# nkb-tech/nkb-classification

Hardware: AMD Instinct MI355X
Metric: images/sec train step (3x224x224) (higher is better)
Workload: dtype bf16; 1 GPU; resnet50 single-task train step, 1000 classes, bs=256/GPU, bf16 compute + fp32 master weights, NAdam, 3x224x224; global_batch=256, parallelism=dp1

## Files before the change

nkb-classification_amd/csrc/elementwise.hip:

```cpp
#include "common.h"
#include <stdlib.h>
#include <atomic>

static inline unsigned grid_for(size_t work_items, int block = 256, unsigned cap = 256 * 16) {
    size_t g = (work_items + block - 1) / block;
    if (g > cap) g = cap;
    if (g < 1) g = 1;
    return (unsigned)g;
}

template <typename T> struct Chunk;
template <> struct Chunk<bf16_t> {
    static constexpr int N = 8;
    __device__ static __forceinline__ void load(const bf16_t* p, float* f) { unpack8(*(const u32x4*)p, f); }
    __device__ static __forceinline__ void store(bf16_t* p, const float* f) { *(u32x4*)p = pack8(f); }
};
template <> struct Chunk<float> {
    static constexpr int N = 4;
    __device__ static __forceinline__ void load(const float* p, float* f) {
        const f32x4 v = *(const f32x4*)p;
        f[0] = v[0]; f[1] = v[1]; f[2] = v[2]; f[3] = v[3];
    }
    __device__ static __forceinline__ void store(float* p, const float* f) { *(f32x4*)p = (f32x4){f[0], f[1], f[2], f[3]}; }
};

static inline int env_int(const char* name, int dflt) {
    const char* v = getenv(name);
    return v && *v ? atoi(v) : dflt;
}
#ifndef NKB_BN_FUSED
#define NKB_BN_FUSED 1
#endif
static constexpr int g_bn_fused = NKB_BN_FUSED;

template <int NC>
__device__ __forceinline__ void ldvec(const float* __restrict__ p, float* o) {
#pragma unroll
    for (int i = 0; i < NC / 4; ++i) {
        const f32x4 v = *(const f32x4*)(p + 4 * i);
        o[4 * i] = v[0]; o[4 * i + 1] = v[1]; o[4 * i + 2] = v[2]; o[4 * i + 3] = v[3];
    }
}

static inline int bn_partitions(int C) { return C <= 128 ? 64 : (C <= 256 ? 32 : 16); }
template <bool WT>
__device__ __forceinline__ void bn_partial_reduce_body(const float* __restrict__ partials, int tiles, int C, double* __restrict__ dpart,
                                                       double (&red)[2][16][64]) {
    const int cx = threadIdx.x & 63, py = threadIdx.x >> 6;
    const int c = blockIdx.x * 64 + cx;
    double s = 0.0, ss = 0.0;
    if (c < C) {
        for (int t = blockIdx.y * 16 + py; t < tiles; t += 16 * (int)gridDim.y) {
            s += (double)partials[((size_t)t * 2) * C + c];
            ss += (double)partials[((size_t)t * 2 + 1) * C + c];
        }
    }
    red[0][py][cx] = s;
    red[1][py][cx] = ss;
    __syncthreads();
    if (py != 0 || c >= C) return;
    s = 0.0; ss = 0.0;
    for (int k = 0; k < 16; ++k) { s += red[0][k][cx]; ss += red[1][k][cx]; }
    double* d0 = dpart + ((size_t)blockIdx.y * 2) * C + c;
    double* d1 = dpart + ((size_t)blockIdx.y * 2 + 1) * C + c;
    if constexpr (WT) {
        __hip_atomic_store(d0, s, __ATOMIC_RELAXED, __HIP_MEMORY_SCOPE_AGENT);
        __hip_atomic_store(d1, ss, __ATOMIC_RELAXED, __HIP_MEMORY_SCOPE_AGENT);
    } else {
        *d0 = s; *d1 = ss;
    }
}
__global__ void bn_partial_reduce_kernel(const float* __restrict__ partials, int tiles, int C, double* __restrict__ dpart) {
    __shared__ double red[2][16][64];
    bn_partial_reduce_body<false>(partials, tiles, C, dpart, red);
}

__device__ unsigned g_bn_tickets[128 * 32];
__device__ __forceinline__ bool bn_arrive_last(unsigned* ticket, unsigned parts) {
    __shared__ unsigned last_flag;
    asm volatile("s_waitcnt vmcnt(0)" ::: "memory");
    __syncthreads();
    if (threadIdx.x == 0) {
        const unsigned t = __hip_atomic_fetch_add(ticket, 1u, __ATOMIC_RELAXED, __HIP_MEMORY_SCOPE_AGENT);
        const bool last = t == parts - 1;
        if (last) {
            __hip_atomic_store(ticket, 0u, __ATOMIC_RELAXED, __HIP_MEMORY_SCOPE_AGENT);
            __builtin_amdgcn_fence(__ATOMIC_ACQUIRE, "agent");
            asm volatile("s_waitcnt vmcnt(0)" ::: "memory");
        }
        last_flag = last ? 1u : 0u;
    }
    __syncthreads();
    return last_flag != 0u;
}
static unsigned* bn_ticket_slot(int cols) {
    static std::atomic<unsigned> next{0};
    if (cols > 32) return nullptr;
    unsigned* base = nullptr;
    if (hipGetSymbolAddress((void**)&base, HIP_SYMBOL(g_bn_tickets)) != hipSuccess || !base) return nullptr;
    return base + (next.fetch_add(1u) % 128u) * 32u;
}

template <typename PT>
__device__ __forceinline__ void bn_finalize_body(const PT* __restrict__ partials, int tiles, int C, float count,
                                                 const float* __restrict__ gamma, const float* __restrict__ beta,
                                                 float* __restrict__ running_mean, float* __restrict__ running_var,
                                                 float momentum, float eps, int training, float* __restrict__ scale,
                                                 float* __restrict__ shift, float* __restrict__ save_mean,
                                                 float* __restrict__ save_invstd, double (&red)[2][16][64]) {
    const int cx = threadIdx.x & 63, py = threadIdx.x >> 6;
    const int c = blockIdx.x * 64 + cx;
    double s = 0.0, ss = 0.0;
    if (training && c < C) {
        for (int t = py; t < tiles; t += 16) {
            s += (double)partials[((size_t)t * 2) * C + c];
            ss += (double)partials[((size_t)t * 2 + 1) * C + c];
        }
    }
    red[0][py][cx] = s;
    red[1][py][cx] = ss;
    __syncthreads();
    if (py != 0 || c >= C) return;
    float mean, var;
    if (training) {
        s = 0.0; ss = 0.0;
        for (int k = 0; k < 16; ++k) { s += red[0][k][cx]; ss += red[1][k][cx]; }
        const double m = s / count;
        double v = ss / count - m * m;
        if (v < 0.0) v = 0.0;
        mean = (float)m; var = (float)v;
        const float unbiased = count > 1.f ? (float)(v * count / (count - 1.0)) : var;
        running_mean[c] = (1.f - momentum) * running_mean[c] + momentum * mean;
        running_var[c] = (1.f - momentum) * running_var[c] + momentum * unbiased;
    } else {
        mean = running_mean[c]; var = running_var[c];
    }
    const float invstd = 1.0f / sqrtf(var + eps);
    const float g = gamma ? gamma[c] : 1.f, b = beta ? beta[c] : 0.f;
    scale[c] = g * invstd;
    shift[c] = b - mean * g * invstd;
    if (save_mean) { save_mean[c] = mean; save_invstd[c] = invstd; }
}
template <typename PT>
__global__ void bn_finalize_kernel(const PT* __restrict__ partials, int tiles, int C, float count,
                                   const float* __restrict__ gamma, const float* __restrict__ beta,
                                   float* __restrict__ running_mean, float* __restrict__ running_var,
                                   float momentum, float eps, int training, float* __restrict__ scale,
                                   float* __restrict__ shift, float* __restrict__ save_mean,
                                   float* __restrict__ save_invstd) {
    __shared__ double red[2][16][64];
    bn_finalize_body<PT>(partials, tiles, C, count, gamma, beta, running_mean, running_var, momentum, eps, training, scale, shift,
                         save_mean, save_invstd, red);
}
__global__ __launch_bounds__(1024) void bn_reduce_finalize_kernel(const float* __restrict__ partials, int tiles, int C, double* __restrict__ dpart,
                                                                  unsigned* __restrict__ tickets, float count,
                                                                  const float* __restrict__ gamma, const float* __restrict__ beta,
                                                                  float* __restrict__ running_mean, float* __restrict__ running_var,
                                                                  float momentum, float eps, float* __restrict__ scale,
                                                                  float* __restrict__ shift, float* __restrict__ save_mean,
                                                                  float* __restrict__ save_invstd) {
    __shared__ double red[2][16][64];
    bn_partial_reduce_body<true>(partials, tiles, C, dpart, red);
    if (!bn_arrive_last(tickets + blockIdx.x, gridDim.y)) return;
    bn_finalize_body<double>(dpart, (int)gridDim.y, C, count, gamma, beta, running_mean, running_var, momentum, eps, 1, scale, shift,
                             save_mean, save_invstd, red);
}

extern "C" int nkb_bn_finalize(const float* partials, int tiles, int C, long long count, const float* gamma,
                               const float* beta, float* running_mean, float* running_var, float momentum, float eps,
                               int training, float* scale, float* shift, float* save_mean, float* save_invstd,
                               hipStream_t stream) {
    NkbProfScope prof(NKB_K_BN_FINALIZE, stream, 0);
    if (training && tiles > 128) {
        double* dpart = (double*)(partials + (((size_t)tiles * 2 * C + 1) & ~(size_t)1));
        const int P = bn_partitions(C);
        unsigned* tickets = g_bn_fused ? bn_ticket_slot((C + 63) / 64) : nullptr;
        if (tickets) {
// ... 637 lines not shown
}
extern "C" int nkb_wprep(int dtype, const float* src, void* dst, int A, int B, int C, int ld, int mode, hipStream_t stream) {
    if (mode < 0 || mode > 5 || (mode >= 2 && B != 9)) { nkb_set_error("wprep: bad mode %d (B=%d)", mode, B); return 1; }
    const size_t total = wprep_total(A, B, C, ld, mode);
    NkbProfScope prof(NKB_K_WPREP, stream, 0);
    if (dtype == NKB_DT_BF16)
        hipLaunchKernelGGL(wprep_kernel<bf16_t>, dim3(grid_for(total)), dim3(256), 0, stream, src, (bf16_t*)dst, A, B, C, ld, mode, total);
    else
        hipLaunchKernelGGL(wprep_kernel<float>, dim3(grid_for(total)), dim3(256), 0, stream, src, (float*)dst, A, B, C, ld, mode, total);
    return nkb_check_launch("wprep");
}

template <typename T>
__global__ void wfold_kernel(const float* __restrict__ w, const float* __restrict__ scale, T* __restrict__ dst, int K, size_t total) {
    for (size_t i = (size_t)blockIdx.x * blockDim.x + threadIdx.x; i < total; i += (size_t)gridDim.x * blockDim.x)
        DT<T>::st(dst + i, w[i] * scale[i / K]);
}
extern "C" int nkb_wfold(int dtype, const float* w, const float* scale, void* dst, int Cout, int K, hipStream_t stream) {
    if (dtype != NKB_DT_BF16 && dtype != NKB_DT_F32) { nkb_set_error("wfold: bad dtype %d", dtype); return 1; }
    if (Cout <= 0 || K <= 0) return 0;
    const size_t total = (size_t)Cout * K;
    NkbProfScope prof(NKB_K_WPREP, stream, 0);
    if (dtype == NKB_DT_BF16) hipLaunchKernelGGL(wfold_kernel<bf16_t>, dim3(grid_for(total)), dim3(256), 0, stream, w, scale, (bf16_t*)dst, K, total);
    else hipLaunchKernelGGL(wfold_kernel<float>, dim3(grid_for(total)), dim3(256), 0, stream, w, scale, (float*)dst, K, total);
    return nkb_check_launch("wfold");
}

template <typename T>
__global__ void splitk_reduce_kernel(const float* __restrict__ partial, int S, int M, int N, T* __restrict__ y, int ldy,
                                     const float* __restrict__ bias, float* __restrict__ stats) {
    const int n = blockIdx.x * blockDim.x + threadIdx.x;
    if (n >= N) return;
    const int m0 = blockIdx.y * 128, m1 = min(M, m0 + 128);
    const float b = bias ? bias[n] : 0.f;
    float s = 0.f, ss = 0.f;
    for (int m = m0; m < m1; ++m) {
        float v = b;
        for (int z = 0; z < S; ++z) v += partial[((size_t)z * M + m) * N + n];
        v = DT<T>::rnd(v);
        DT<T>::st(y + (size_t)m * ldy + n, v);
        s += v; ss += v * v;
    }
    if (stats) {
        stats[((size_t)blockIdx.y * 2) * N + n] = s;
        stats[((size_t)blockIdx.y * 2 + 1) * N + n] = ss;
    }
}
template <typename T>
__global__ void splitk_reduce4_kernel(const float* __restrict__ partial, int S, int M, int N, T* __restrict__ y, int ldy,
                                      const float* __restrict__ bias) {
    const int n4 = N >> 2;
    const size_t i = (size_t)blockIdx.x * blockDim.x + threadIdx.x;
    if (i >= (size_t)M * n4) return;
    const int m = (int)(i / n4), c = (int)(i - (size_t)m * n4) * 4;
    f32x4 v = bias ? *(const f32x4*)(bias + c) : (f32x4){0.f, 0.f, 0.f, 0.f};
    const float* p = partial + (size_t)m * N + c;
    const size_t slab = (size_t)M * N;
    for (int z = 0; z < S; ++z) v += *(const f32x4*)(p + (size_t)z * slab);
#pragma unroll
    for (int e = 0; e < 4; ++e) DT<T>::st(y + (size_t)m * ldy + c + e, DT<T>::rnd(v[e]));
}
template <typename T>
__global__ void splitk_stats_kernel(const T* __restrict__ y, int M, int N, int ldy, float* __restrict__ stats) {
    const int n = blockIdx.x * blockDim.x + threadIdx.x;
    if (n >= N) return;
    const int m0 = blockIdx.y * 128, m1 = min(M, m0 + 128);
    float s = 0.f, ss = 0.f;
    for (int m = m0; m < m1; ++m) { const float v = DT<T>::ld(y + (size_t)m * ldy + n); s += v; ss += v * v; }
    stats[((size_t)blockIdx.y * 2) * N + n] = s;
    stats[((size_t)blockIdx.y * 2 + 1) * N + n] = ss;
}
extern "C" int nkb_splitk_reduce(int dtype, const float* partial, int splits, int M, int N, void* y, int ldy, const float* bias,
                                 float* stats, hipStream_t stream) {
    if (dtype != NKB_DT_BF16 && dtype != NKB_DT_F32) { nkb_set_error("splitk_reduce: bad dtype %d", dtype); return 1; }
    if (splits < 1 || M < 1 || N < 1 || ldy < N) { nkb_set_error("splitk_reduce: bad shape"); return 1; }
    NkbProfScope prof(NKB_K_MISC, stream, 0);
    if (N % 4 == 0 && (((size_t)bias) & 15) == 0) {
        const size_t total = (size_t)M * (N >> 2);
        const dim3 g4((unsigned)((total + 255) / 256)), gs((N + 255) / 256, (M + 127) / 128);
        if (dtype == NKB_DT_BF16) {
            hipLaunchKernelGGL(splitk_reduce4_kernel<bf16_t>, g4, dim3(256), 0, stream, partial, splits, M, N, (bf16_t*)y, ldy, bias);
            if (stats) hipLaunchKernelGGL(splitk_stats_kernel<bf16_t>, gs, dim3(256), 0, stream, (const bf16_t*)y, M, N, ldy, stats);
        } else {
            hipLaunchKernelGGL(splitk_reduce4_kernel<float>, g4, dim3(256), 0, stream, partial, splits, M, N, (float*)y, ldy, bias);
            if (stats) hipLaunchKernelGGL(splitk_stats_kernel<float>, gs, dim3(256), 0, stream, (const float*)y, M, N, ldy, stats);
        }
        return nkb_check_launch("splitk_reduce");
    }
    dim3 grid((N + 255) / 256, (M + 127) / 128);
    if (dtype == NKB_DT_BF16) hipLaunchKernelGGL(splitk_reduce_kernel<bf16_t>, grid, dim3(256), 0, stream, partial, splits, M, N, (bf16_t*)y, ldy, bias, stats);
    else hipLaunchKernelGGL(splitk_reduce_kernel<float>, grid, dim3(256), 0, stream, partial, splits, M, N, (float*)y, ldy, bias, stats);
    return nkb_check_launch("splitk_reduce");
}

__global__ void add2d_kernel(const float* __restrict__ src, float* __restrict__ dst, int rows, int cols, int ld_src, int ld_dst) {
    const size_t total = (size_t)rows * cols;
    for (size_t i = (size_t)blockIdx.x * blockDim.x + threadIdx.x; i < total; i += (size_t)gridDim.x * blockDim.x) {
        const int c = (int)(i % cols), r = (int)(i / cols);
        dst[(size_t)r * ld_dst + c] += src[(size_t)r * ld_src + c];
    }
}
extern "C" int nkb_add2d(const float* src, float* dst, int rows, int cols, int ld_src, int ld_dst, hipStream_t stream) {
    NkbProfScope prof(NKB_K_MISC, stream, 0);
    hipLaunchKernelGGL(add2d_kernel, dim3(grid_for((size_t)rows * cols)), dim3(256), 0, stream, src, dst, rows, cols, ld_src, ld_dst);
    return nkb_check_launch("add2d");
}

template <typename T>
__global__ void colsum_kernel(const T* __restrict__ x, float* __restrict__ out, int rows, int C, int ld) {
    const int c = blockIdx.x * 64 + (threadIdx.x & 63);
    const int part = threadIdx.x >> 6;
    __shared__ float red[4][64];
    float t = 0.f;
    if (c < C) for (int r = part; r < rows; r += 4) t += DT<T>::ld(x + (size_t)r * ld + c);
    red[part][threadIdx.x & 63] = t;
    __syncthreads();
    if (part == 0 && c < C) out[c] += red[0][threadIdx.x] + red[1][threadIdx.x] + red[2][threadIdx.x] + red[3][threadIdx.x];
}
extern "C" int nkb_colsum(int dtype, const void* x, float* out, int rows, int C, int ld, hipStream_t stream) {
    NkbProfScope prof(NKB_K_MISC, stream, 0);
    if (dtype == NKB_DT_BF16) hipLaunchKernelGGL(colsum_kernel<bf16_t>, dim3((C + 63) / 64), dim3(256), 0, stream, (const bf16_t*)x, out, rows, C, ld);
    else hipLaunchKernelGGL(colsum_kernel<float>, dim3((C + 63) / 64), dim3(256), 0, stream, (const float*)x, out, rows, C, ld);
    return nkb_check_launch("colsum");
}

template <typename T>
__global__ void pad_cast_kernel(const float* __restrict__ src, T* __restrict__ dst, int rows, int C, int ld_src, int ld_dst, float mul) {
    const size_t total = (size_t)rows * ld_dst;
    for (size_t i = (size_t)blockIdx.x * blockDim.x + threadIdx.x; i < total; i += (size_t)gridDim.x * blockDim.x) {
        const int c = (int)(i % ld_dst), r = (int)(i / ld_dst);
        DT<T>::st(dst + i, c < C ? src[(size_t)r * ld_src + c] * mul : 0.f);
    }
}
extern "C" int nkb_pad_cast(int dtype, const float* src, void* dst, int rows, int C, int ld_src, int ld_dst, float mul, hipStream_t stream) {
    NkbProfScope prof(NKB_K_MISC, stream, 0);
    const size_t total = (size_t)rows * ld_dst;
    if (dtype == NKB_DT_BF16) hipLaunchKernelGGL(pad_cast_kernel<bf16_t>, dim3(grid_for(total)), dim3(256), 0, stream, src, (bf16_t*)dst, rows, C, ld_src, ld_dst, mul);
    else hipLaunchKernelGGL(pad_cast_kernel<float>, dim3(grid_for(total)), dim3(256), 0, stream, src, (float*)dst, rows, C, ld_src, ld_dst, mul);
    return nkb_check_launch("pad_cast");
}

template <int NC> struct SlotWord;
template <> struct SlotWord<8> {
    unsigned long long w;
    __device__ __forceinline__ void load(const unsigned char* p) { w = *(const unsigned long long*)p; }
    __device__ __forceinline__ int get(int e) const { return (int)((w >> (8 * e)) & 0xff); }
};
template <> struct SlotWord<4> {
    unsigned w;
    __device__ __forceinline__ void load(const unsigned char* p) { w = *(const unsigned*)p; }
    __device__ __forceinline__ int get(int e) const { return (int)((w >> (8 * e)) & 0xff); }
};

template <typename T>
__global__ __launch_bounds__(256) void bn_relu_maxpool_fwd_kernel(const T* __restrict__ c, const float* __restrict__ scale,
                                                                  const float* __restrict__ shift, T* __restrict__ y,
                                                                  unsigned char* __restrict__ idx, T* __restrict__ xsel, int N,
                                                                  int H, int W, int C, int P, int Q) {
    constexpr int NC = Chunk<T>::N;
    const unsigned cpr = (unsigned)C / NC;
    const unsigned t = blockIdx.x * blockDim.x + threadIdx.x;
    const unsigned cg = t % cpr, pstride = (gridDim.x * blockDim.x) / cpr;
    const unsigned npix = (unsigned)N * P * Q;
    float sc[NC], sh[NC];
    ldvec<NC>(scale + cg * NC, sc);
    ldvec<NC>(shift + cg * NC, sh);
    for (unsigned pix = t / cpr; pix < npix; pix += pstride) {
        const unsigned q = pix % (unsigned)Q, pn = pix / (unsigned)Q;
        const unsigned pp = pn % (unsigned)P, n = pn / (unsigned)P;
        float best[NC], bx[NC];
        int bi[NC];
#pragma unroll
        for (int e = 0; e < NC; ++e) { best[e] = -INFINITY; bi[e] = 0; bx[e] = 0.f; }
        bool first = true;
        for (int r = 0; r < 3; ++r) {
            const int h = 2 * (int)pp - 1 + r;
            if ((unsigned)h >= (unsigned)H) continue;
            for (int s = 0; s < 3; ++s) {
                const int w = 2 * (int)q - 1 + s;
                if ((unsigned)w >= (unsigned)W) continue;
                float v[NC];
                Chunk<T>::load(c + (((size_t)n * H + h) * W + w) * C + cg * NC, v);
#pragma unroll
                for (int e = 0; e < NC; ++e) {
                    const float a = DT<T>::rnd(fmaxf(v[e] * sc[e] + sh[e], 0.f));
                    if (first || a > best[e] || a != a) { best[e] = a; bi[e] = r * 3 + s; bx[e] = v[e]; }
                }
                first = false;
            }
        }
        const size_t o = (size_t)pix * C + cg * NC;
        Chunk<T>::store(y + o, best);
        if (xsel) Chunk<T>::store(xsel + o, bx);
        unsigned long long word = 0;
#pragma unroll
        for (int e = 0; e < NC; ++e) word |= (unsigned long long)bi[e] << (8 * e);
        if (NC == 8) *(unsigned long long*)(idx + o) = word;
        else *(unsigned*)(idx + o) = (unsigned)word;
    }
}

template <typename T>
__global__ void bn_relu_maxpool_bwd_reduce_kernel(const T* __restrict__ g, const unsigned char* __restrict__ idx,
                                                  const T* __restrict__ c, const float* __restrict__ scale,
                                                  const float* __restrict__ shift, const float* __restrict__ mean,
                                                  const float* __restrict__ invstd, const T* __restrict__ xsel, int N, int H,
                                                  int W, int C, int P, int Q, int rpb, float* __restrict__ part) {
    constexpr int NC = Chunk<T>::N;
    extern __shared__ float red[];
    const int cpr = C / NC;
    const int tpc = blockDim.x / cpr;
    const int cg = threadIdx.x % cpr, rl = threadIdx.x / cpr;
    float s1[NC], s2[NC];
#pragma unroll
    for (int e = 0; e < NC; ++e) { s1[e] = 0.f; s2[e] = 0.f; }
    const long long rows = (long long)N * P * Q;
    if (rl < tpc) {
        float sc[NC], sh[NC], mu[NC], is[NC];
        ldvec<NC>(scale + cg * NC, sc);
        ldvec<NC>(shift + cg * NC, sh);
        ldvec<NC>(mean + cg * NC, mu);
        ldvec<NC>(invstd + cg * NC, is);
        for (long long r = (long long)blockIdx.x * tpc + rl; r < rows; r += (long long)gridDim.x * tpc) {
            const unsigned ru = (unsigned)r;
            const int q = (int)(ru % (unsigned)Q);
            const unsigned pn = ru / (unsigned)Q;
            const int pp = (int)(pn % (unsigned)P);
            const int n = (int)(pn / (unsigned)P);
            const size_t o = (size_t)r * C + cg * NC;
            float gv[NC];
            Chunk<T>::load(g + o, gv);
            SlotWord<NC> sw;
            sw.load(idx + o);
            const T* cbase = c + (((size_t)n * H + (2 * pp - 1)) * W + (2 * q - 1)) * C + cg * NC;
            float xs[NC];
            if (xsel) Chunk<T>::load(xsel + o, xs);
#pragma unroll
            for (int e = 0; e < NC; ++e) {
                float x;
                if (xsel) x = xs[e];
                else {
                    const int slot = sw.get(e);
                    const int dr = (slot * 11) >> 5;
                    const int ds = slot - 3 * dr;
                    x = DT<T>::ld(cbase + ((ptrdiff_t)dr * W + ds) * C + e);
                }
                if (DT<T>::rnd(x * sc[e] + sh[e]) > 0.f) { s1[e] += gv[e]; s2[e] += gv[e] * (x - mu[e]) * is[e]; }
            }
        }
#pragma unroll
        for (int e = 0; e < NC; ++e) {
            red[(0 * tpc + rl) * C + cg * NC + e] = s1[e];
            red[(1 * tpc + rl) * C + cg * NC + e] = s2[e];
        }
    }
    __syncthreads();
    for (int i = threadIdx.x; i < 2 * C; i += blockDim.x) {
        const int which = i / C, ch = i % C;
        float t = 0.f;
        for (int k = 0; k < tpc; ++k) t += red[(which * tpc + k) * C + ch];
        part[((size_t)blockIdx.x * 2 + which) * C + ch] = t;
    }
}

template <typename T>
__global__ __launch_bounds__(256) void bn_relu_maxpool_bwd_apply_kernel(
    const T* __restrict__ g, const unsigned char* __restrict__ idx, const T* __restrict__ c,
    const float* __restrict__ scale, const float* __restrict__ shift, const float* __restrict__ mean,
    const float* __restrict__ invstd, const float* __restrict__ gamma, const float* __restrict__ sums, float inv_count,
    T* __restrict__ dc, int N, int H, int W, int C, int P, int Q) {
    constexpr int NC = Chunk<T>::N;
    const unsigned cpr = (unsigned)C / NC;
    const unsigned t = blockIdx.x * blockDim.x + threadIdx.x;
    const unsigned cg = t % cpr, pstride = (gridDim.x * blockDim.x) / cpr;
    const unsigned npix = (unsigned)N * H * W;
    float k1[NC], k2[NC], k3[NC], fs[NC], fb[NC], v_is[NC], v_ga[NC], v_mu[NC], v_s1[NC], v_s2[NC];
    ldvec<NC>(scale + cg * NC, fs);
    ldvec<NC>(shift + cg * NC, fb);
    ldvec<NC>(invstd + cg * NC, v_is);
    ldvec<NC>(mean + cg * NC, v_mu);
    ldvec<NC>(sums + cg * NC, v_s1);
    ldvec<NC>(sums + C + cg * NC, v_s2);
    if (gamma) ldvec<NC>(gamma + cg * NC, v_ga);
#pragma unroll
    for (int e = 0; e < NC; ++e) {
        const float is = v_is[e], ga = gamma ? v_ga[e] : 1.f, mu = v_mu[e];
        const float a = ga * is;
        const float sdy = v_s1[e] * inv_count, sdyx = v_s2[e] * inv_count;
        k1[e] = a;
        k2[e] = -a * is * sdyx;
        k3[e] = -a * sdy + a * is * sdyx * mu;
    }
    for (unsigned pix = t / cpr; pix < npix; pix += pstride) {
        const unsigned w = pix % (unsigned)W, hn = pix / (unsigned)W;
        const unsigned h = hn % (unsigned)H, n = hn / (unsigned)H;
        float acc[NC], xv[NC], out[NC];
        const size_t ofs = (size_t)pix * C + cg * NC;
        Chunk<T>::load(c + ofs, xv);
#pragma unroll
        for (int e = 0; e < NC; ++e) acc[e] = 0.f;
        const int p0 = h >> 1, p1 = (h + 1) >> 1, q0 = w >> 1, q1 = (w + 1) >> 1;
        float gv[4][NC];
        SlotWord<NC> sw[4];
        int slot[4];
        bool ok[4];
#pragma unroll
        for (int k = 0; k < 4; ++k) {
            const int pp = (k >> 1) ? p1 : p0, q = (k & 1) ? q1 : q0;
            ok[k] = pp < P && q < Q && !((k >> 1) && p1 == p0) && !((k & 1) && q1 == q0);
            const int pc = pp < P ? pp : P - 1, qc = q < Q ? q : Q - 1;
            slot[k] = ((int)h - (2 * pp - 1)) * 3 + ((int)w - (2 * q - 1));
            const size_t o = ((((size_t)n * P + pc) * Q + qc) * C) + cg * NC;
            Chunk<T>::load(g + o, gv[k]);
            sw[k].load(idx + o);
        }
#pragma unroll
        for (int k = 0; k < 4; ++k)
#pragma unroll
            for (int e = 0; e < NC; ++e) if (ok[k] && sw[k].get(e) == slot[k]) acc[e] += gv[k][e];
#pragma unroll
        for (int e = 0; e < NC; ++e) {
            float gg = acc[e];
            if (!(DT<T>::rnd(xv[e] * fs[e] + fb[e]) > 0.f)) gg = 0.f;
            out[e] = k1[e] * gg + (k2[e] * xv[e] + k3[e]);
        }
        Chunk<T>::store(dc + ofs, out);
    }
}

extern "C" int nkb_bn_relu_maxpool_sel(int dtype, int backward, const void* c, const float* scale, const float* shift,
                                       const float* mean, const float* invstd, const float* gamma, void* y_or_g,
                                       unsigned char* idx, void* dc, float* dgamma, float* dbeta, float* workspace,
                                       size_t workspace_floats, void* xsel, int N, int H, int W, int C, hipStream_t stream);
extern "C" int nkb_bn_relu_maxpool(int dtype, int backward, const void* c, const float* scale, const float* shift,
                                   const float* mean, const float* invstd, const float* gamma, void* y_or_g,
                                   unsigned char* idx, void* dc, float* dgamma, float* dbeta, float* workspace,
                                   size_t workspace_floats, int N, int H, int W, int C, hipStream_t stream) {
    return nkb_bn_relu_maxpool_sel(dtype, backward, c, scale, shift, mean, invstd, gamma, y_or_g, idx, dc, dgamma, dbeta, workspace,
                                   workspace_floats, nullptr, N, H, W, C, stream);
}
extern "C" int nkb_bn_relu_maxpool_sel(int dtype, int backward, const void* c, const float* scale, const float* shift,
                                       const float* mean, const float* invstd, const float* gamma, void* y_or_g,
                                       unsigned char* idx, void* dc, float* dgamma, float* dbeta, float* workspace,
                                       size_t workspace_floats, void* xsel, int N, int H, int W, int C, hipStream_t stream) {
    const int P = (H + 2 - 3) / 2 + 1, Q = (W + 2 - 3) / 2 + 1;
    const int n = dtype == NKB_DT_BF16 ? 8 : 4;
    if (C % n || C / n > 256) { nkb_set_error("bn_relu_maxpool: unsupported C=%d", C); return 1; }
    if ((long long)N * H * W >= (1ll << 31)) { nkb_set_error("bn_relu_maxpool: N*H*W too large"); return 1; }
    if (!backward) {
        NkbProfScope prof(NKB_K_MAXPOOL, stream, 0);
        const unsigned grid = grid_cols((size_t)N * P * Q, C / n);
        if (dtype == NKB_DT_BF16)
            hipLaunchKernelGGL(bn_relu_maxpool_fwd_kernel<bf16_t>, dim3(grid), dim3(256), 0, stream,
                               (const bf16_t*)c, scale, shift, (bf16_t*)y_or_g, idx, (bf16_t*)xsel, N, H, W, C, P, Q);
        else
            hipLaunchKernelGGL(bn_relu_maxpool_fwd_kernel<float>, dim3(grid), dim3(256), 0, stream,
                               (const float*)c, scale, shift, (float*)y_or_g, idx, (float*)xsel, N, H, W, C, P, Q);
        return nkb_check_launch("bn_relu_maxpool_fwd");
    }
    const long long rows = (long long)N * P * Q;
    const int cpr = C / n;
    const int tpc = 256 / cpr;
    int blocks = (int)((rows + 63) / 64);
    if (blocks > 1024) blocks = 1024;
    if (blocks < 1) blocks = 1;
    const int rpb = (int)((rows + blocks - 1) / blocks);
    blocks = (int)((rows + rpb - 1) / rpb);
    const size_t need = (size_t)blocks * 2 * C + 2 * C;
    if (workspace_floats < need) { nkb_set_error("bn_relu_maxpool: workspace %zu < %zu floats", workspace_floats, need); return 1; }
    float* part = workspace;
    float* sums = workspace + (size_t)blocks * 2 * C;
    const size_t lds = (size_t)2 * tpc * C * sizeof(float);
    {
        NkbProfScope prof(NKB_K_BN_BWD_REDUCE, stream, 0);
        if (dtype == NKB_DT_BF16)
            hipLaunchKernelGGL(bn_relu_maxpool_bwd_reduce_kernel<bf16_t>, dim3(blocks), dim3(256), lds, stream,
                               (const bf16_t*)y_or_g, idx, (const bf16_t*)c, scale, shift, mean, invstd, (const bf16_t*)xsel, N, H, W, C, P, Q,
                               rpb, part);
        else
            hipLaunchKernelGGL(bn_relu_maxpool_bwd_reduce_kernel<float>, dim3(blocks), dim3(256), lds, stream,
                               (const float*)y_or_g, idx, (const float*)c, scale, shift, mean, invstd, (const float*)xsel, N, H, W, C, P, Q,
                               rpb, part);
        hipLaunchKernelGGL(bn_bwd_finalize_kernel, dim3((C + 15) / 16), dim3(1024), 0, stream, part, blocks, C, dgamma, dbeta, sums);
    }
    if (int rc = nkb_check_launch("bn_relu_maxpool_bwd_reduce")) return rc;
    {
        NkbProfScope prof(NKB_K_BN_BWD_APPLY, stream, 0);
        const unsigned grid = grid_cols((size_t)N * H * W, cpr);
        const float inv_count = 1.0f / (float)((long long)N * H * W);
        if (dtype == NKB_DT_BF16)
            hipLaunchKernelGGL(bn_relu_maxpool_bwd_apply_kernel<bf16_t>, dim3(grid), dim3(256), 0, stream,
                               (const bf16_t*)y_or_g, idx, (const bf16_t*)c, scale, shift, mean, invstd, gamma, sums, inv_count,
                               (bf16_t*)dc, N, H, W, C, P, Q);
        else
            hipLaunchKernelGGL(bn_relu_maxpool_bwd_apply_kernel<float>, dim3(grid), dim3(256), 0, stream,
                               (const float*)y_or_g, idx, (const float*)c, scale, shift, mean, invstd, gamma, sums, inv_count,
                               (float*)dc, N, H, W, C, P, Q);
    }
    return nkb_check_launch("bn_relu_maxpool_bwd_apply");
}

extern "C" size_t nkb_bn_relu_maxpool_workspace_floats(int N, int H, int W, int C) {
    const long long P = (H + 2 - 3) / 2 + 1, Q = (W + 2 - 3) / 2 + 1;
    long long blocks = ((long long)N * P * Q + 63) / 64;
    if (blocks > 1024) blocks = 1024;
    if (blocks < 1) blocks = 1;
    return (size_t)blocks * 2 * C + 2 * C;
}

template <typename T>
__global__ void stem_pack_kernel(const float* __restrict__ x, T* __restrict__ out, int N, int C, int H, int W, int Wp) {
    const size_t total = (size_t)N * H * Wp;
    for (size_t i = (size_t)blockIdx.x * blockDim.x + threadIdx.x; i < total; i += (size_t)gridDim.x * blockDim.x) {
        const int w = (int)(i % Wp);
        const size_t nh = i / Wp;
        const size_t n = nh / H, h = nh - n * H;
        float v[4] = {0.f, 0.f, 0.f, 0.f};
        if (w < W)
            for (int c = 0; c < C; ++c) v[c] = x[((n * C + c) * H + h) * W + w];
        if constexpr (sizeof(T) == 2) {
            u32x2 o = {pack_bf2(v[0], v[1]), pack_bf2(v[2], v[3])};
            *(u32x2*)(out + i * 4) = o;
        } else {
            *(f32x4*)(out + i * 4) = (f32x4){v[0], v[1], v[2], v[3]};
        }
    }
}
extern "C" int nkb_stem_pack(int dtype, const float* x, void* out, int N, int C, int H, int W, hipStream_t stream) {
    if (C < 1 || C > 4) { nkb_set_error("stem_pack: C=%d outside 1..4", C); return 1; }
    NkbProfScope prof(NKB_K_IM2COL, stream, 0);
    const int Wp = (W + 1) & ~1;
    const size_t total = (size_t)N * H * Wp;
    if (dtype == NKB_DT_BF16) hipLaunchKernelGGL(stem_pack_kernel<bf16_t>, dim3(grid_for(total)), dim3(256), 0, stream, x, (bf16_t*)out, N, C, H, W, Wp);
    else hipLaunchKernelGGL(stem_pack_kernel<float>, dim3(grid_for(total)), dim3(256), 0, stream, x, (float*)out, N, C, H, W, Wp);
    return nkb_check_launch("stem_pack");
}

__device__ __forceinline__ bool stem_col_to_tap(int col, int epc, int cprw, int lead, int& r, int& s, int& ch) {
    const int j = col % epc, sc = (col / epc) % cprw;
    r = col / (epc * cprw);
    s = sc * (epc / 4) + j / 4 - lead;
    ch = j % 4;
    return r < 7 && s >= 0 && s < 7;
}
template <typename T>
__global__ void stem_weight_kernel(const float* __restrict__ src, T* __restrict__ wp, float* __restrict__ dw, int Cout,
                                   int C, int cols, int epc, int cprw, int lead, int fold) {
    const int total = Cout * cols;
    for (int i = blockIdx.x * blockDim.x + threadIdx.x; i < total; i += gridDim.x * blockDim.x) {
        const int co = i / cols, col = i - co * cols;
        int r, s, ch;
        const bool ok = stem_col_to_tap(col, epc, cprw, lead, r, s, ch) && ch < C;
        const int widx = ((co * 7 + r) * 7 + s) * C + ch;
        if (fold) { if (ok) dw[widx] += src[i]; }
        else DT<T>::st(wp + i, ok ? src[widx] : 0.f);
    }
}
extern "C" int nkb_stem_wprep(int dtype, const float* w, void* wp, int Cout, int C, hipStream_t stream) {
    const int epc = dtype == NKB_DT_BF16 ? 8 : 4, cprw = dtype == NKB_DT_BF16 ? 4 : 8, lead = dtype == NKB_DT_BF16 ? 1 : 0;
    const int rpt = 8 / cprw, cols = (7 + rpt - 1) / rpt * 8 * epc;
    NkbProfScope prof(NKB_K_WPREP, stream, 0);
    if (dtype == NKB_DT_BF16) hipLaunchKernelGGL(stem_weight_kernel<bf16_t>, dim3(grid_for((size_t)Cout * cols)), dim3(256), 0, stream, w, (bf16_t*)wp, nullptr, Cout, C, cols, epc, cprw, lead, 0);
    else hipLaunchKernelGGL(stem_weight_kernel<float>, dim3(grid_for((size_t)Cout * cols)), dim3(256), 0, stream, w, (float*)wp, nullptr, Cout, C, cols, epc, cprw, lead, 0);
    return nkb_check_launch("stem_wprep");
}
extern "C" int nkb_stem_wfold(int dtype, const float* dwp, float* dw, int Cout, int C, hipStream_t stream) {
    const int epc = dtype == NKB_DT_BF16 ? 8 : 4, cprw = dtype == NKB_DT_BF16 ? 4 : 8, lead = dtype == NKB_DT_BF16 ? 1 : 0;
    const int cols = 7 * cprw * epc;
    NkbProfScope prof(NKB_K_MISC, stream, 0);
    hipLaunchKernelGGL(stem_weight_kernel<float>, dim3(grid_for((size_t)Cout * cols)), dim3(256), 0, stream, dwp, nullptr, dw, Cout, C, cols, epc, cprw, lead, 1);
    return nkb_check_launch("stem_wfold");
}

template <typename PT>
__device__ __forceinline__ void bn_bwd_finalize_tiles_body(const PT* __restrict__ partials, int tiles, int C,
                                                           const float* __restrict__ invstd, float* __restrict__ dgamma,
                                                           float* __restrict__ dbeta, float* __restrict__ sums, double (&red)[2][16][64]) {
    const int cx = threadIdx.x & 63, py = threadIdx.x >> 6;
    const int c = blockIdx.x * 64 + cx;
    double a = 0.0, b = 0.0;
    if (c < C) {
        for (int t = py; t < tiles; t += 16) {
            a += (double)partials[((size_t)t * 2) * C + c];
            b += (double)partials[((size_t)t * 2 + 1) * C + c];
        }
    }
    red[0][py][cx] = a;
    red[1][py][cx] = b;
    __syncthreads();
    if (py != 0 || c >= C) return;
    a = 0.0; b = 0.0;
    for (int k = 0; k < 16; ++k) { a += red[0][k][cx]; b += red[1][k][cx]; }
    const float sg = (float)a, sgx = (float)(b * (invstd ? (double)invstd[c] : 1.0));
    sums[c] = sg;
    sums[C + c] = sgx;
    if (dbeta) dbeta[c] += sg;
    if (dgamma) dgamma[c] += sgx;
}
template <typename PT>
__global__ void bn_bwd_finalize_tiles_kernel(const PT* __restrict__ partials, int tiles, int C,
                                             const float* __restrict__ invstd, float* __restrict__ dgamma,
                                             float* __restrict__ dbeta, float* __restrict__ sums) {
    __shared__ double red[2][16][64];
    bn_bwd_finalize_tiles_body<PT>(partials, tiles, C, invstd, dgamma, dbeta, sums, red);
}
__global__ __launch_bounds__(1024) void bn_bwd_reduce_finalize_kernel(const float* __restrict__ stats, int tiles, int C, double* __restrict__ dpart,
                                                                      unsigned* __restrict__ tickets, const float* __restrict__ invstd,
                                                                      float* __restrict__ dgamma, float* __restrict__ dbeta,
                                                                      float* __restrict__ sums) {
    __shared__ double red[2][16][64];
    bn_partial_reduce_body<true>(stats, tiles, C, dpart, red);
    if (!bn_arrive_last(tickets + blockIdx.x, gridDim.y)) return;
    bn_bwd_finalize_tiles_body<double>(dpart, (int)gridDim.y, C, invstd, dgamma, dbeta, sums, red);
}

static void launch_bwd_tile_sums(float* stats, int tiles, int C, const float* invstd, float* dgamma, float* dbeta, float* sums,
                                 hipStream_t stream) {
    double* dpart = (double*)(stats + (((size_t)tiles * 2 * C + 1) & ~(size_t)1));
    const int P = bn_partitions(C);
    unsigned* tickets = g_bn_fused ? bn_ticket_slot((C + 63) / 64) : nullptr;
    if (tickets) {
        hipLaunchKernelGGL(bn_bwd_reduce_finalize_kernel, dim3((C + 63) / 64, P), dim3(1024), 0, stream, stats, tiles, C, dpart, tickets,
                           invstd, dgamma, dbeta, sums);
        return;
    }
    hipLaunchKernelGGL(bn_partial_reduce_kernel, dim3((C + 63) / 64, P), dim3(1024), 0, stream, stats, tiles, C, dpart);
    hipLaunchKernelGGL(bn_bwd_finalize_tiles_kernel<double>, dim3((C + 63) / 64), dim3(1024), 0, stream,
                       (const double*)dpart, P, C, invstd, dgamma, dbeta, sums);
}

int nkb_launch_tile_sums(float* stats, int tiles, int C, float* sums, hipStream_t stream) {
    if (tiles > 128) {
        launch_bwd_tile_sums(stats, tiles, C, nullptr, nullptr, nullptr, sums, stream);
    } else {
        hipLaunchKernelGGL(bn_bwd_finalize_tiles_kernel<float>, dim3((C + 63) / 64), dim3(1024), 0, stream,
                           (const float*)stats, tiles, C, (const float*)nullptr, (float*)nullptr, (float*)nullptr, sums);
    }
    return nkb_check_launch("tile_sums");
}

extern "C" int nkb_bn_backward_from_stats(int dtype, const void* g, const void* x, float* stats, int tiles,
                                          const float* mean, const float* invstd, const float* gamma, long long rows,
                                          int C, float* dgamma, float* dbeta, void* dx, float* sums, hipStream_t stream) {
    const int n = dtype == NKB_DT_BF16 ? 8 : 4;
    if (C % n || rows >= (1ll << 31)) { nkb_set_error("bn_backward_from_stats: unsupported C=%d / rows", C); return 1; }
    {
        NkbProfScope prof(NKB_K_BN_BWD_REDUCE, stream, 0);
        if (tiles > 128) {
            launch_bwd_tile_sums(stats, tiles, C, invstd, dgamma, dbeta, sums, stream);
        } else {
// ... 18 lines not shown
```

Before: 14990 images/sec.

## Tile stem BN-ReLU-maxpool fwd/bwd kernels over row bands to reuse loads

Rewrites the fused BN+ReLU+maxpool forward kernel so each thread handles a band of output rows and a run of output columns. The shared input row between adjacent pooling windows is reduced once and carried forward instead of reloaded, and the argmax value and slot are packed into a single word for bf16. The backward apply kernel is likewise restructured to process 2x4 input pixel tiles per thread across row bands, reusing gradient and index loads across neighbouring pixels. Both kernels get occupancy hints and loads pinned early for latency hiding. In exchange the kernels use more registers, and the grid is sized per work unit rather than grid-strided.

```diff
diff --git a/nkb-classification_amd/csrc/elementwise.hip b/nkb-classification_amd/csrc/elementwise.hip
--- a/nkb-classification_amd/csrc/elementwise.hip
+++ b/nkb-classification_amd/csrc/elementwise.hip
@@ -12,17 +12,26 @@
 template <typename T> struct Chunk;
 template <> struct Chunk<bf16_t> {
     static constexpr int N = 8;
+    using Raw = u32x4;
+    __device__ static __forceinline__ Raw ldraw(const bf16_t* p) { return *(const u32x4*)p; }
+    __device__ static __forceinline__ void unpack(const Raw& r, float* f) { unpack8(r, f); }
     __device__ static __forceinline__ void load(const bf16_t* p, float* f) { unpack8(*(const u32x4*)p, f); }
     __device__ static __forceinline__ void store(bf16_t* p, const float* f) { *(u32x4*)p = pack8(f); }
 };
 template <> struct Chunk<float> {
     static constexpr int N = 4;
+    using Raw = f32x4;
+    __device__ static __forceinline__ Raw ldraw(const float* p) { return *(const f32x4*)p; }
+    __device__ static __forceinline__ void unpack(const Raw& r, float* f) { f[0] = r[0]; f[1] = r[1]; f[2] = r[2]; f[3] = r[3]; }
     __device__ static __forceinline__ void load(const float* p, float* f) {
         const f32x4 v = *(const f32x4*)p;
         f[0] = v[0]; f[1] = v[1]; f[2] = v[2]; f[3] = v[3];
     }
     __device__ static __forceinline__ void store(float* p, const float* f) { *(f32x4*)p = (f32x4){f[0], f[1], f[2], f[3]}; }
 };
+
+template <typename V>
+__device__ __forceinline__ void pin_load(V& v) { asm volatile("" : "+v"(v)); }
 
 static inline int env_int(const char* name, int dflt) {
     const char* v = getenv(name);
@@ -966,51 +975,141 @@
     __device__ __forceinline__ int get(int e) const { return (int)((w >> (8 * e)) & 0xff); }
 };
 
-template <typename T>
-__global__ __launch_bounds__(256) void bn_relu_maxpool_fwd_kernel(const T* __restrict__ c, const float* __restrict__ scale,
+constexpr int PF_QR = 2, PF_PB = 6;
+
+template <typename T> struct Picked;
+template <> struct Picked<bf16_t> {
+    unsigned w;
+    __device__ static __forceinline__ Picked make(float x, int slot) { return {__float_as_uint(x) | (unsigned)slot}; }
+    __device__ static __forceinline__ Picked sel(bool t, Picked a, Picked b) { return {t ? a.w : b.w}; }
+    __device__ __forceinline__ Picked plus(int d) const { return {w + (unsigned)d}; }
+    __device__ __forceinline__ int slot() const { return (int)(w & 15u); }
+    __device__ __forceinline__ float x() const { return __uint_as_float(w & 0xffff0000u); }
+};
+template <> struct Picked<float> {
+    float v; int s;
+    __device__ static __forceinline__ Picked make(float x, int slot) { return {x, slot}; }
+    __device__ static __forceinline__ Picked sel(bool t, Picked a, Picked b) { return {t ? a.v : b.v, t ? a.s : b.s}; }
+    __device__ __forceinline__ Picked plus(int d) const { return {v, s + d}; }
+    __device__ __forceinline__ int slot() const { return s; }
+    __device__ __forceinline__ float x() const { return v; }
+};
+
+template <typename T, int QR>
+struct PoolRow { float a[QR][Chunk<T>::N]; Picked<T> px[QR][Chunk<T>::N]; };
+
+template <typename T, int QR>
+__device__ __forceinline__ void pool_row_reduce(const float (&v)[2 * QR + 1][Chunk<T>::N], const bool (&wok)[2 * QR + 1],
+                                                const float* sc, const float* sh, PoolRow<T, QR>& row) {
+    constexpr int NC = Chunk<T>::N;
+    float a[2 * QR + 1][NC];
+#pragma unroll
+    for (int j = 0; j < 2 * QR + 1; ++j)
+#pragma unroll
+        for (int e = 0; e < NC; ++e)
+            a[j][e] = DT<T>::rnd(fmaxf(v[j][e] * sc[e] + sh[e], 0.f));
+#pragma unroll
+    for (int k = 0; k < QR; ++k) {
+        bool first = true;
+#pragma unroll
+        for (int e = 0; e < NC; ++e) { row.a[k][e] = -INFINITY; row.px[k][e] = Picked<T>::make(0.f, 0); }
+#pragma unroll
+        for (int s = 0; s < 3; ++s) {
+            const int j = 2 * k + s;
+#pragma unroll
+            for (int e = 0; e < NC; ++e) {
+                const bool take = wok[j] & (first | (a[j][e] > row.a[k][e]));
+                row.a[k][e] = take ? a[j][e] : row.a[k][e];
+                row.px[k][e] = Picked<T>::sel(take, Picked<T>::make(v[j][e], s), row.px[k][e]);
+            }
+            first = first & !wok[j];
+        }
+    }
+}
+
+template <typename T>
+__global__ __launch_bounds__(256, 3) void bn_relu_maxpool_fwd_kernel(const T* __restrict__ c, const float* __restrict__ scale,
                                                                   const float* __restrict__ shift, T* __restrict__ y,
                                                                   unsigned char* __restrict__ idx, T* __restrict__ xsel, int N,
-                                                                  int H, int W, int C, int P, int Q) {
-    constexpr int NC = Chunk<T>::N;
+                                                                  int H, int W, int C, int P, int Q, int runs, int bands,
+                                                                  size_t nunits) {
+    constexpr int NC = Chunk<T>::N, QR = PF_QR, NCOL = 2 * QR + 1;
     const unsigned cpr = (unsigned)C / NC;
-    const unsigned t = blockIdx.x * blockDim.x + threadIdx.x;
-    const unsigned cg = t % cpr, pstride = (gridDim.x * blockDim.x) / cpr;
-    const unsigned npix = (unsigned)N * P * Q;
+    const size_t t = (size_t)blockIdx.x * blockDim.x + threadIdx.x;
+    const unsigned cg = (unsigned)(t % cpr);
+    const size_t unit = t / cpr;
+    if (unit >= nunits) return;
+    const int run = (int)(unit % (unsigned)runs);
+    const size_t nb = unit / (unsigned)runs;
+    const int band = (int)(nb % (unsigned)bands), n = (int)(nb / (unsigned)bands);
+    const int q0 = run * QR, p0 = band * PF_PB, p1 = p0 + PF_PB < P ? p0 + PF_PB : P;
     float sc[NC], sh[NC];
     ldvec<NC>(scale + cg * NC, sc);
     ldvec<NC>(shift + cg * NC, sh);
-    for (unsigned pix = t / cpr; pix < npix; pix += pstride) {
-        const unsigned q = pix % (unsigned)Q, pn = pix / (unsigned)Q;
-        const unsigned pp = pn % (unsigned)P, n = pn / (unsigned)P;
-        float best[NC], bx[NC];
-        int bi[NC];
-#pragma unroll
-        for (int e = 0; e < NC; ++e) { best[e] = -INFINITY; bi[e] = 0; bx[e] = 0.f; }
-        bool first = true;
-        for (int r = 0; r < 3; ++r) {
-            const int h = 2 * (int)pp - 1 + r;
-            if ((unsigned)h >= (unsigned)H) continue;
-            for (int s = 0; s < 3; ++s) {
-                const int w = 2 * (int)q - 1 + s;
-                if ((unsigned)w >= (unsigned)W) continue;
-                float v[NC];
-                Chunk<T>::load(c + (((size_t)n * H + h) * W + w) * C + cg * NC, v);
-#pragma unroll
-                for (int e = 0; e < NC; ++e) {
-                    const float a = DT<T>::rnd(fmaxf(v[e] * sc[e] + sh[e], 0.f));
-                    if (first || a > best[e] || a != a) { best[e] = a; bi[e] = r * 3 + s; bx[e] = v[e]; }
-                }
-                first = false;
+    bool wok[NCOL];
+    unsigned wof[NCOL];
+#pragma unroll
+    for (int j = 0; j < NCOL; ++j) {
+        const int w = 2 * q0 - 1 + j;
+        wok[j] = (unsigned)w < (unsigned)W;
+        wof[j] = (unsigned)(w < 0 ? 0 : (w < W ? w : W - 1)) * C + cg * NC;
+    }
+    const T* img = c + (size_t)n * H * W * C;
+    typename Chunk<T>::Raw rm[NCOL], rb[NCOL];
+    float v[NCOL][NC];
+    PoolRow<T, QR> top, mid, bot;
+    bool top_ok = p0 > 0;
+    {
+        const T* pt = img + (size_t)(top_ok ? 2 * p0 - 1 : 0) * W * C;
+#pragma unroll
+        for (int j = 0; j < NCOL; ++j) rm[j] = Chunk<T>::ldraw(pt + wof[j]);
+#pragma unroll
+        for (int j = 0; j < NCOL; ++j) { pin_load(rm[j]); Chunk<T>::unpack(rm[j], v[j]); }
+        pool_row_reduce<T, QR>(v, wok, sc, sh, top);
+    }
+    for (int p = p0; p < p1; ++p) {
+        const bool bot_ok = 2 * p + 1 < H;
+        const T* pm = img + (size_t)(2 * p) * W * C;
+        const T* pb = img + (size_t)(bot_ok ? 2 * p + 1 : H - 1) * W * C;
+#pragma unroll
+        for (int j = 0; j < NCOL; ++j) rm[j] = Chunk<T>::ldraw(pm + wof[j]);
+#pragma unroll
+        for (int j = 0; j < NCOL; ++j) rb[j] = Chunk<T>::ldraw(pb + wof[j]);
+#pragma unroll
+        for (int j = 0; j < NCOL; ++j) { pin_load(rm[j]); Chunk<T>::unpack(rm[j], v[j]); }
+        pool_row_reduce<T, QR>(v, wok, sc, sh, mid);
+#pragma unroll
+        for (int j = 0; j < NCOL; ++j) { pin_load(rb[j]); Chunk<T>::unpack(rb[j], v[j]); }
+        pool_row_reduce<T, QR>(v, wok, sc, sh, bot);
+#pragma unroll
+        for (int k = 0; k < QR; ++k) {
+            float best[NC], bx[NC];
+            int bi[NC];
+#pragma unroll
+            for (int e = 0; e < NC; ++e) {
+                const float ma = mid.a[k][e], ba = bot.a[k][e];
+                const bool take_mid = !top_ok | (ma > top.a[k][e]);
+                best[e] = take_mid ? ma : top.a[k][e];
+                Picked<T> px = Picked<T>::sel(take_mid, mid.px[k][e].plus(3), top.px[k][e]);
+                const bool take_bot = bot_ok & (ba > best[e]);
+                best[e] = take_bot ? ba : best[e];
+                px = Picked<T>::sel(take_bot, bot.px[k][e].plus(6), px);
+                bi[e] = px.slot();
+                bx[e] = px.x();
             }
-        }
-        const size_t o = (size_t)pix * C + cg * NC;
-        Chunk<T>::store(y + o, best);
-        if (xsel) Chunk<T>::store(xsel + o, bx);
-        unsigned long long word = 0;
-#pragma unroll
-        for (int e = 0; e < NC; ++e) word |= (unsigned long long)bi[e] << (8 * e);
-        if (NC == 8) *(unsigned long long*)(idx + o) = word;
-        else *(unsigned*)(idx + o) = (unsigned)word;
+            if (q0 + k < Q) {
+                const size_t o = ((((size_t)n * P + p) * Q + (q0 + k)) * C) + cg * NC;
+                Chunk<T>::store(y + o, best);
+                if (xsel) Chunk<T>::store(xsel + o, bx);
+                unsigned long long word = 0;
+#pragma unroll
+                for (int e = 0; e < NC; ++e) word |= (unsigned long long)bi[e] << (8 * e);
+                if (NC == 8) *(unsigned long long*)(idx + o) = word;
+                else *(unsigned*)(idx + o) = (unsigned)word;
+            }
+        }
+        top = bot;
+        top_ok = bot_ok;
     }
 }
 
@@ -1077,17 +1176,24 @@
     }
 }
 
-template <typename T>
-__global__ __launch_bounds__(256) void bn_relu_maxpool_bwd_apply_kernel(
+constexpr int PB_RP = 6;
+
+template <typename T>
+__global__ __launch_bounds__(256, 3) void bn_relu_maxpool_bwd_apply_kernel(
     const T* __restrict__ g, const unsigned char* __restrict__ idx, const T* __restrict__ c,
     const float* __restrict__ scale, const float* __restrict__ shift, const float* __restrict__ mean,
     const float* __restrict__ invstd, const float* __restrict__ gamma, const float* __restrict__ sums, float inv_count,
-    T* __restrict__ dc, int N, int H, int W, int C, int P, int Q) {
+    T* __restrict__ dc, int N, int H, int W, int C, int P, int Q, int strips, int bands, size_t nunits) {
     constexpr int NC = Chunk<T>::N;
     const unsigned cpr = (unsigned)C / NC;
-    const unsigned t = blockIdx.x * blockDim.x + threadIdx.x;
-    const unsigned cg = t % cpr, pstride = (gridDim.x * blockDim.x) / cpr;
-    const unsigned npix = (unsigned)N * H * W;
+    const size_t t = (size_t)blockIdx.x * blockDim.x + threadIdx.x;
+    const unsigned cg = (unsigned)(t % cpr);
+    const size_t unit = t / cpr;
+    if (unit >= nunits) return;
+    const int u = (int)(unit % (unsigned)strips);
+    const size_t nb = unit / (unsigned)strips;
+    const int band = (int)(nb % (unsigned)bands), n = (int)(nb / (unsigned)bands);
+    const int pairs = (H + 1) / 2, i0 = band * PB_RP, i1 = i0 + PB_RP < pairs ? i0 + PB_RP : pairs;
     float k1[NC], k2[NC], k3[NC], fs[NC], fb[NC], v_is[NC], v_ga[NC], v_mu[NC], v_s1[NC], v_s2[NC];
     ldvec<NC>(scale + cg * NC, fs);
     ldvec<NC>(shift + cg * NC, fb);
@@ -1105,40 +1211,63 @@
         k2[e] = -a * is * sdyx;
         k3[e] = -a * sdy + a * is * sdyx * mu;
     }
-    for (unsigned pix = t / cpr; pix < npix; pix += pstride) {
-        const unsigned w = pix % (unsigned)W, hn = pix / (unsigned)W;
-        const unsigned h = hn % (unsigned)H, n = hn / (unsigned)H;
-        float acc[NC], xv[NC], out[NC];
-        const size_t ofs = (size_t)pix * C + cg * NC;
-        Chunk<T>::load(c + ofs, xv);
-#pragma unroll
-        for (int e = 0; e < NC; ++e) acc[e] = 0.f;
-        const int p0 = h >> 1, p1 = (h + 1) >> 1, q0 = w >> 1, q1 = (w + 1) >> 1;
-        float gv[4][NC];
-        SlotWord<NC> sw[4];
-        int slot[4];
-        bool ok[4];
-#pragma unroll
-        for (int k = 0; k < 4; ++k) {
-            const int pp = (k >> 1) ? p1 : p0, q = (k & 1) ? q1 : q0;
-            ok[k] = pp < P && q < Q && !((k >> 1) && p1 == p0) && !((k & 1) && q1 == q0);
-            const int pc = pp < P ? pp : P - 1, qc = q < Q ? q : Q - 1;
-            slot[k] = ((int)h - (2 * pp - 1)) * 3 + ((int)w - (2 * q - 1));
-            const size_t o = ((((size_t)n * P + pc) * Q + qc) * C) + cg * NC;
-            Chunk<T>::load(g + o, gv[k]);
-            sw[k].load(idx + o);
-        }
-#pragma unroll
-        for (int k = 0; k < 4; ++k)
-#pragma unroll
-            for (int e = 0; e < NC; ++e) if (ok[k] && sw[k].get(e) == slot[k]) acc[e] += gv[k][e];
-#pragma unroll
-        for (int e = 0; e < NC; ++e) {
-            float gg = acc[e];
-            if (!(DT<T>::rnd(xv[e] * fs[e] + fb[e]) > 0.f)) gg = 0.f;
-            out[e] = k1[e] * gg + (k2[e] * xv[e] + k3[e]);
-        }
-        Chunk<T>::store(dc + ofs, out);
+    const int w0 = 4 * u, qb = 2 * u;
+    unsigned wof[4], qof[3];
+#pragma unroll
+    for (int j = 0; j < 4; ++j) wof[j] = (unsigned)(w0 + j < W ? w0 + j : W - 1) * C + cg * NC;
+#pragma unroll
+    for (int j = 0; j < 3; ++j) qof[j] = (unsigned)(qb + j < Q ? qb + j : Q - 1) * C + cg * NC;
+    const size_t img = (size_t)n * H * W * C, pimg = (size_t)n * P * Q * C;
+    typename Chunk<T>::Raw gr[2][3], xr[2][4];
+    SlotWord<NC> sw[2][3];
+    {
+        const size_t o = pimg + (size_t)i0 * Q * C;
+#pragma unroll
+        for (int j = 0; j < 3; ++j) { gr[0][j] = Chunk<T>::ldraw(g + o + qof[j]); sw[0][j].load(idx + o + qof[j]); }
+    }
+    for (int i = i0; i < i1; ++i) {
+        {
+            const size_t o = pimg + (size_t)(i + 1 < P ? i + 1 : P - 1) * Q * C;
+#pragma unroll
+            for (int j = 0; j < 3; ++j) { gr[1][j] = Chunk<T>::ldraw(g + o + qof[j]); sw[1][j].load(idx + o + qof[j]); }
+        }
+#pragma unroll
+        for (int dh = 0; dh < 2; ++dh) {
+            const size_t o = img + (size_t)(2 * i + dh < H ? 2 * i + dh : H - 1) * W * C;
+#pragma unroll
+            for (int dw = 0; dw < 4; ++dw) xr[dh][dw] = Chunk<T>::ldraw(c + o + wof[dw]);
+        }
+        float gv[2][3][NC];
+#pragma unroll
+        for (int pr = 0; pr < 2; ++pr)
+#pragma unroll
+            for (int j = 0; j < 3; ++j) { pin_load(gr[pr][j]); pin_load(sw[pr][j].w); Chunk<T>::unpack(gr[pr][j], gv[pr][j]); }
+#pragma unroll
+        for (int dh = 0; dh < 2; ++dh)
+#pragma unroll
+            for (int dw = 0; dw < 4; ++dw) {
+                float acc[NC], out[NC], xv[NC];
+                pin_load(xr[dh][dw]);
+                Chunk<T>::unpack(xr[dh][dw], xv);
+#pragma unroll
+                for (int e = 0; e < NC; ++e) acc[e] = 0.f;
+#pragma unroll
+                for (int k = 0; k < 4; ++k) {
+                    const int pr = (k >> 1) ? dh : 0, qj = (k & 1) ? (dw + 1) >> 1 : dw >> 1;
+                    const bool ok = i + pr < P && qb + qj < Q && !((k >> 1) && dh == 0) && !((k & 1) && (dw & 1) == 0);
+                    const int slot = (dh + 1 - 2 * pr) * 3 + (dw + 1 - 2 * qj);
+#pragma unroll
+                    for (int e = 0; e < NC; ++e) acc[e] = (ok & (sw[pr][qj].get(e) == slot)) ? acc[e] + gv[pr][qj][e] : acc[e];
+                }
+#pragma unroll
+                for (int e = 0; e < NC; ++e) {
+                    const float gg = DT<T>::rnd(xv[e] * fs[e] + fb[e]) > 0.f ? acc[e] : 0.f;
+                    out[e] = k1[e] * gg + (k2[e] * xv[e] + k3[e]);
+                }
+                if (2 * i + dh < H && w0 + dw < W) Chunk<T>::store(dc + img + (size_t)(2 * i + dh) * W * C + wof[dw], out);
+            }
+#pragma unroll
+        for (int j = 0; j < 3; ++j) { gr[0][j] = gr[1][j]; sw[0][j] = sw[1][j]; }
     }
 }
 
@@ -1161,15 +1290,18 @@
     const int n = dtype == NKB_DT_BF16 ? 8 : 4;
     if (C % n || C / n > 256) { nkb_set_error("bn_relu_maxpool: unsupported C=%d", C); return 1; }
     if ((long long)N * H * W >= (1ll << 31)) { nkb_set_error("bn_relu_maxpool: N*H*W too large"); return 1; }
+    if ((long long)W * C >= (1ll << 31)) { nkb_set_error("bn_relu_maxpool: W*C too large"); return 1; }
     if (!backward) {
         NkbProfScope prof(NKB_K_MAXPOOL, stream, 0);
-        const unsigned grid = grid_cols((size_t)N * P * Q, C / n);
+        const int runs = (Q + PF_QR - 1) / PF_QR, bands = (P + PF_PB - 1) / PF_PB;
+        const size_t nunits = (size_t)N * bands * runs;
+        const unsigned grid = (unsigned)((nunits * (C / n) + 255) / 256);
         if (dtype == NKB_DT_BF16)
             hipLaunchKernelGGL(bn_relu_maxpool_fwd_kernel<bf16_t>, dim3(grid), dim3(256), 0, stream,
-                               (const bf16_t*)c, scale, shift, (bf16_t*)y_or_g, idx, (bf16_t*)xsel, N, H, W, C, P, Q);
+                               (const bf16_t*)c, scale, shift, (bf16_t*)y_or_g, idx, (bf16_t*)xsel, N, H, W, C, P, Q, runs, bands, nunits);
         else
             hipLaunchKernelGGL(bn_relu_maxpool_fwd_kernel<float>, dim3(grid), dim3(256), 0, stream,
-                               (const float*)c, scale, shift, (float*)y_or_g, idx, (float*)xsel, N, H, W, C, P, Q);
+                               (const float*)c, scale, shift, (float*)y_or_g, idx, (float*)xsel, N, H, W, C, P, Q, runs, bands, nunits);
         return nkb_check_launch("bn_relu_maxpool_fwd");
     }
     const long long rows = (long long)N * P * Q;
@@ -1200,16 +1332,18 @@
     if (int rc = nkb_check_launch("bn_relu_maxpool_bwd_reduce")) return rc;
     {
         NkbProfScope prof(NKB_K_BN_BWD_APPLY, stream, 0);
-        const unsigned grid = grid_cols((size_t)N * H * W, cpr);
+        const int strips = (W + 3) / 4, abands = ((H + 1) / 2 + PB_RP - 1) / PB_RP;
+        const size_t nunits = (size_t)N * abands * strips;
+        const unsigned grid = (unsigned)((nunits * cpr + 255) / 256);
         const float inv_count = 1.0f / (float)((long long)N * H * W);
         if (dtype == NKB_DT_BF16)
             hipLaunchKernelGGL(bn_relu_maxpool_bwd_apply_kernel<bf16_t>, dim3(grid), dim3(256), 0, stream,
                                (const bf16_t*)y_or_g, idx, (const bf16_t*)c, scale, shift, mean, invstd, gamma, sums, inv_count,
-                               (bf16_t*)dc, N, H, W, C, P, Q);
+                               (bf16_t*)dc, N, H, W, C, P, Q, strips, abands, nunits);
         else
             hipLaunchKernelGGL(bn_relu_maxpool_bwd_apply_kernel<float>, dim3(grid), dim3(256), 0, stream,
                                (const float*)y_or_g, idx, (const float*)c, scale, shift, mean, invstd, gamma, sums, inv_count,
-                               (float*)dc, N, H, W, C, P, Q);
+                               (float*)dc, N, H, W, C, P, Q, strips, abands, nunits);
     }
     return nkb_check_launch("bn_relu_maxpool_bwd_apply");
 }
```

New measurement: 15120 images/sec (median of 6 runs). No clear change (+0.9%).
